# sephiroce/srf

Measured on AMD Instinct MI355X. Metric: acoustic frames/sec through SRF (123-d fbank, 3-iter DR) at 1/2/4/8 MI355X, higher is better.
Workload: dtype fp32; 1 GPU; wsj_c4: SRF L=6 PH=CH=16 DIM=32 LPAD=RPAD=2 DR iter=3, train step (fwd+bwd+allreduce+Adam); utterances_per_gpu=28, frames_per_utterance=800, global_batch=28, parallelism=dp1, launch=hipgraph (fwd+CTC+bwd)

## Files before the change

### srf_amd/csrc/cnnfe.hip

```cpp
#include <algorithm>
#include <type_traits>
#include <cmath>
#include <cstdlib>

#include "srf_common.h"
#include "srf_reduce.h"
#include "srf_rng.h"
#include "../../include/srf.h"

namespace {

constexpr int C = 64;
constexpr float kBnEps = 1e-3f;
constexpr float kBnMomentum = 0.99f;

struct Dims {
  int B, T, Fin;
  int T1, F1, T2, F2;
  int pt1, pf1, pt2, pf2;
};

inline int same_out(int n) { return (n + 1) / 2; }
inline int same_pad_before(int n) {
  const int out = same_out(n);
  const int total = std::max((out - 1) * 2 + 3 - n, 0);
  return total / 2;
}

Dims make_dims(int B, int T, int Fin) {
  Dims d;
  d.B = B; d.T = T; d.Fin = Fin;
  d.T1 = same_out(T); d.F1 = same_out(Fin);
  d.T2 = same_out(d.T1); d.F2 = same_out(d.F1);
  d.pt1 = same_pad_before(T); d.pf1 = same_pad_before(Fin);
  d.pt2 = same_pad_before(d.T1); d.pf2 = same_pad_before(d.F1);
  return d;
}

__device__ __forceinline__ int ceil_div_len(int len, int div) { return (len + div - 1) / div; }

__device__ __forceinline__ void chan_merge(float& n, float& mean, float& m2, float nb, float meanb, float m2b) {
  if (nb == 0.f) return;
  const float nn = n + nb;
  const float delta = meanb - mean;
  mean += delta * (nb / nn);
  m2 += m2b + delta * delta * (n * nb / nn);
  n = nn;
}

constexpr int kPackW2Threads = 2 * C * 64;
constexpr int kPackW2tThreads = 9 * C * (2 * C / 8);
__device__ __forceinline__ void pack_w2_f16_body(int idx, const float* __restrict__ ka, const float* __restrict__ kb,
                                                 _Float16* __restrict__ wp2, float* __restrict__ wsc);
__device__ __forceinline__ void pack_w2t_split_body(int idx, const float* __restrict__ ka,
                                                    const float* __restrict__ kb, __bf16* __restrict__ wq3);
__device__ __forceinline__ void pack_w2t_f16_body(int idx, const float* __restrict__ ka, const float* __restrict__ kb,
                                                  _Float16* __restrict__ wq2h, float* __restrict__ wdsc);
constexpr int kPackW2tF16Threads = C * 64;

constexpr int kRows1 = 4;

struct Tile1 {
  int b, t1_0, fpad;
};

__device__ __forceinline__ Tile1 stage_rows1(const float* __restrict__ feats, const Dims& d, float* win) {
  const int tiles_per_b = (d.T1 + kRows1 - 1) / kRows1;
  Tile1 tl;
  tl.b = blockIdx.x / tiles_per_b;
  tl.t1_0 = (blockIdx.x - tl.b * tiles_per_b) * kRows1;
  tl.fpad = d.Fin + 2;
  const int nrows = 2 * kRows1 + 1;
  const int t_base = 2 * tl.t1_0 - d.pt1;
  for (int k = threadIdx.x; k < nrows * tl.fpad; k += blockDim.x) {
    const int r = k / tl.fpad, col = k - r * tl.fpad;
    const int t = t_base + r, f = col - 1;
    const bool ok = t >= 0 && t < d.T && f >= 0 && f < d.Fin;
    const float v = feats[((size_t)tl.b * d.T + min(max(t, 0), d.T - 1)) * d.Fin + min(max(f, 0), d.Fin - 1)];
    win[k] = ok ? v : 0.f;
  }
  __syncthreads();
  return tl;
}

__device__ __forceinline__ void window9_lds(const float* win, const Tile1& tl, const Dims& d, int w, int f1,
                                            float (&x)[9]) {
#pragma unroll
  for (int dt = 0; dt < 3; ++dt)
#pragma unroll
    for (int df = 0; df < 3; ++df) x[dt * 3 + df] = win[(2 * w + dt) * tl.fpad + 2 * f1 - d.pf1 + df + 1];
}

__global__ __launch_bounds__(256) void conv1_fwd_kernel(
    const float* __restrict__ feats, const int* __restrict__ inp_len, Dims d, const float* __restrict__ ka,
    const float* __restrict__ ba, const float* __restrict__ kb, const float* __restrict__ bb, int training,
    float drop_p, unsigned long long seed, const unsigned long long* __restrict__ seed_src, float* __restrict__ y1, unsigned char* __restrict__ sel1,
    float* __restrict__ part, int nconv, const float* __restrict__ pk_a, const float* __restrict__ pk_b,
    _Float16* __restrict__ wp2, float* __restrict__ wsc, float* __restrict__ ymax) {
  if ((int)blockIdx.x >= nconv) {
    const int idx = (blockIdx.x - nconv) * blockDim.x + threadIdx.x;
    if (idx < kPackW2Threads) pack_w2_f16_body(idx, pk_a, pk_b, wp2, wsc);
    return;
  }
  seed = srf_step_seed(seed, seed_src);
  extern __shared__ __attribute__((aligned(16))) float win[];
  __shared__ float sh[3][kRows1][C];
  const int c = threadIdx.x & (C - 1);
  const int w = __builtin_amdgcn_readfirstlane(threadIdx.x >> 6);
  float wa[9], wb[9];
#pragma unroll
  for (int k = 0; k < 9; ++k) {
    wa[k] = ka[k * C + c];
    wb[k] = kb[k * C + c];
  }
  const float bia = ba[c], bib = bb[c];
  const float keep_scale = 1.f / (1.f - drop_p);
  const bool drop = training && drop_p > 0.f;
  const Tile1 tl = stage_rows1(feats, d, win);
  const int t1 = tl.t1_0 + w;
  float n = 0.f, s1 = 0.f, s2 = 0.f, ym = 0.f;
  const float K = 0.5f * (bia + bib);
  if (t1 < d.T1) {
    const bool live = t1 < ceil_div_len(inp_len[tl.b], 2);
    const int pbase = (tl.b * d.T1 + t1) * d.F1;
#pragma unroll 2
    for (int f1 = 0; f1 < d.F1; ++f1) {
      float x[9];
      window9_lds(win, tl, d, w, f1, x);
      float a = bia, bv = bib;
#pragma unroll
      for (int k = 0; k < 9; ++k) {
        a += x[k] * wa[k];
        bv += x[k] * wb[k];
      }
      const int o = (pbase + f1) * C + c;
      if (drop) {
        bool ka, kb;
        srf_keep2(seed, kStreamConv0a, o, drop_p, ka, kb);
        a *= ka ? keep_scale : 0.f;
        bv *= kb ? keep_scale : 0.f;
      }
      const bool sl = a >= bv;
      const float y = live ? (sl ? a : bv) : 0.f;
      y1[o] = y;
      sel1[o] = sl ? 1 : 0;
      ym = fmaxf(ym, fabsf(y));
      n += 1.f;
      s1 += y - K;
      s2 += (y - K) * (y - K);
    }
  }
  float mean = n > 0.f ? K + s1 / n : 0.f;
  float m2 = n > 0.f ? fmaxf(s2 - s1 * s1 / n, 0.f) : 0.f;
  sh[0][w][c] = n; sh[1][w][c] = mean; sh[2][w][c] = m2;
#pragma unroll
  for (int o = 32; o >= 1; o >>= 1) ym = fmaxf(ym, __shfl_xor(ym, o, 64));
  __shared__ float smax[kRows1];
  if (c == 0) smax[w] = ym;
  __syncthreads();
  if (w == 0) {
    if (c == 0) {
      float m = smax[0];
      for (int r = 1; r < kRows1; ++r) m = fmaxf(m, smax[r]);
      ymax[blockIdx.x] = m;
    }
    for (int r = 1; r < kRows1; ++r) chan_merge(n, mean, m2, sh[0][r][c], sh[1][r][c], sh[2][r][c]);
    part[((size_t)blockIdx.x * 3 + 0) * C + c] = n;
    part[((size_t)blockIdx.x * 3 + 1) * C + c] = mean;
    part[((size_t)blockIdx.x * 3 + 2) * C + c] = m2;
  }
}

__global__ __launch_bounds__(256) void bn_merge_kernel(const float* __restrict__ part, int nparts, int per,
                                                       float* __restrict__ out) {
  __shared__ float sh[3][4][C];
  const int c = threadIdx.x & (C - 1), r = threadIdx.x >> 6;
  const int k0 = blockIdx.x * per, k1 = min(nparts, k0 + per);
  float n = 0.f, mu = 0.f, m2 = 0.f;
  for (int k = k0 + r; k < k1; k += 4)
    chan_merge(n, mu, m2, part[((size_t)k * 3 + 0) * C + c], part[((size_t)k * 3 + 1) * C + c],
               part[((size_t)k * 3 + 2) * C + c]);
  sh[0][r][c] = n; sh[1][r][c] = mu; sh[2][r][c] = m2;
  __syncthreads();
  if (r != 0) return;
  for (int q = 1; q < 4; ++q) chan_merge(n, mu, m2, sh[0][q][c], sh[1][q][c], sh[2][q][c]);
  out[((size_t)blockIdx.x * 3 + 0) * C + c] = n;
  out[((size_t)blockIdx.x * 3 + 1) * C + c] = mu;
  out[((size_t)blockIdx.x * 3 + 2) * C + c] = m2;
}

__global__ __launch_bounds__(1024) void bn_finalize_kernel(const float* __restrict__ part, int nparts,
                                                           const float* __restrict__ gamma,
                                                           const float* __restrict__ beta,
                                                           float* __restrict__ mmean, float* __restrict__ mvar,
                                                           int training, float* __restrict__ stats,
                                                           const float* __restrict__ ymax, int nymax) {
  __shared__ float sh[3][16][C];
  __shared__ float ysh[16], ab[2][C];
  const int c = threadIdx.x & (C - 1), r = threadIdx.x >> 6;
  if (ymax != nullptr) {
    float m = 0.f;
    for (int k = threadIdx.x; k < nymax; k += 1024) m = fmaxf(m, ymax[k]);
#pragma unroll
    for (int o = 32; o >= 1; o >>= 1) m = fmaxf(m, __shfl_xor(m, o, 64));
    if (c == 0) ysh[r] = m;
  }
  float n = 0.f, mu = 0.f, m2 = 0.f;
  if (training)
#pragma unroll 8
    for (int k = r; k < nparts; k += 16)
      chan_merge(n, mu, m2, part[((size_t)k * 3 + 0) * C + c], part[((size_t)k * 3 + 1) * C + c],
                 part[((size_t)k * 3 + 2) * C + c]);
  sh[0][r][c] = n; sh[1][r][c] = mu; sh[2][r][c] = m2;
  __syncthreads();
  if (r == 0) {
    float mean, var;
    if (training) {
      for (int q = 1; q < 16; ++q) chan_merge(n, mu, m2, sh[0][q][c], sh[1][q][c], sh[2][q][c]);
      mean = mu;
      var = m2 / n;
      mmean[c] = mmean[c] * kBnMomentum + mean * (1.f - kBnMomentum);
      mvar[c] = mvar[c] * kBnMomentum + (n > 1.f ? var * n / (n - 1.f) : var) * (1.f - kBnMomentum);
    } else {
      mean = mmean[c];
      var = mvar[c];
    }
    const float rstd = 1.f / sqrtf(var + kBnEps);
    const float scale = gamma[c] * rstd;
    const float shift = beta[c] - mean * scale;
    stats[0 * C + c] = mean;
    stats[1 * C + c] = rstd;
    stats[2 * C + c] = scale;
    stats[3 * C + c] = shift;
    ab[0][c] = fabsf(scale);
    ab[1][c] = fabsf(shift);
  }
  if (ymax == nullptr) return;
  __syncthreads();
  if (threadIdx.x == 0) {
    float y = ysh[0], sa = 0.f, sb = 0.f;
    for (int q = 1; q < 16; ++q) y = fmaxf(y, ysh[q]);
    for (int q = 0; q < C; ++q) {
      sa = fmaxf(sa, ab[0][q]);
      sb = fmaxf(sb, ab[1][q]);
    }
    const int e = srf_split_exp(sa * y + sb);
    stats[4 * C + 0] = srf_exp2i(e);
    stats[4 * C + 1] = srf_exp2i(-e);
  }
}

typedef __bf16 cbf8 __attribute__((ext_vector_type(8)));
typedef float cf16 __attribute__((ext_vector_type(16)));

__device__ __forceinline__ cf16 mfma32bf(const cbf8& a, const cbf8& b, const cf16& c) {
  return __builtin_amdgcn_mfma_f32_32x32x16_bf16(a, b, c, 0, 0, 0);
}
typedef _Float16 ch8 __attribute__((ext_vector_type(8)));
__device__ __forceinline__ cf16 mfma32h(const ch8& a, const ch8& b, const cf16& c) {
  return __builtin_amdgcn_mfma_f32_32x32x16_f16(a, b, c, 0, 0, 0);
}

__device__ __forceinline__ void split8v(const float (&v)[8], cbf8& p1, cbf8& p2, cbf8& p3) {
#pragma unroll
  for (int k = 0; k < 8; ++k) {
    const __bf16 a1 = (__bf16)v[k];
    const float r = v[k] - (float)a1;
    const __bf16 a2 = (__bf16)r;
    p1[k] = a1;
    p2[k] = a2;
    p3[k] = (__bf16)(r - (float)a2);
  }
}

__device__ __forceinline__ void pack_w2_f16_body(int idx, const float* __restrict__ ka, const float* __restrict__ kb,
                                                 _Float16* __restrict__ wp2, float* __restrict__ wsc) {
  const int n = idx >> 6, cin = idx & 63;
  const float* k = n < C ? ka : kb;
  const int co = n % C;
  float v[9], m = 0.f;
#pragma unroll
  for (int tap = 0; tap < 9; ++tap) {
    v[tap] = k[((size_t)tap * C + cin) * C + co];
    m = fmaxf(m, fabsf(v[tap]));
  }
#pragma unroll
  for (int o = 32; o >= 1; o >>= 1) m = fmaxf(m, __shfl_xor(m, o, 64));
  const int e = srf_split_exp(m);
  const float sc = srf_exp2i(e);
  const size_t plane = (size_t)9 * 2 * C * C;
#pragma unroll
  for (int tap = 0; tap < 9; ++tap) {
    _Float16 h1, h2;
    srf_split2h(v[tap] * sc, h1, h2);
    const size_t o = ((size_t)tap * 2 * C + n) * C + cin;
    wp2[o] = h1;
    wp2[plane + o] = h2;
  }
  if (cin == 0) wsc[n] = srf_exp2i(-e);
}

constexpr int kC2BStride = 24;
constexpr int kC2Waves = 4;
constexpr int kC2Px = 32 * kC2Waves;
constexpr int kC2BLoads = 2 * 2 * C * 2 / (64 * kC2Waves);

__global__ __launch_bounds__(64 * kC2Waves) __attribute__((amdgpu_waves_per_eu(2))) void conv2_fwd32_kernel(
    const float* __restrict__ y1, const float* __restrict__ stats1, const int* __restrict__ inp_len, Dims d,
    const _Float16* __restrict__ wp2, const float* __restrict__ wsc, const float* __restrict__ ba,
    const float* __restrict__ bb, int training, float drop_p, unsigned long long seed,
    const unsigned long long* __restrict__ seed_src, float* __restrict__ y2, unsigned char* __restrict__ sel2,
    float* __restrict__ part) {
  seed = srf_step_seed(seed, seed_src);
  __shared__ __attribute__((aligned(16))) _Float16 Bs[2][2][2 * C * kC2BStride];
  __shared__ __attribute__((aligned(16))) float ss[2][C];
  __shared__ float red[3][kC2Waves][2 * 32];
  const int tid = threadIdx.x;
  const int lane = tid & 63, wv = tid >> 6;
  const int r = lane & 31, h = lane >> 5;
  const int P2 = d.B * d.T2 * d.F2;
  const int p0 = blockIdx.x * kC2Px;
  const size_t plane = (size_t)9 * 2 * C * C;
  if (tid < 2 * C) ss[tid >> 6][tid & 63] = stats1[(2 + (tid >> 6)) * C + (tid & 63)] * stats1[4 * C];

  const int pa = p0 + 32 * wv + r;
  const bool alive = pa < P2;
  const int pc = min(pa, P2 - 1);
  const int af2 = pc % d.F2, at2 = (pc / d.F2) % d.T2, ab = pc / (d.F2 * d.T2);
  const int alen1 = ceil_div_len(inp_len[ab], 2);

  auto load_b = [&](int kk, ch8 (&bv)[kC2BLoads]) {
    const int tap = kk >> 2, kb = kk & 3;
#pragma unroll
    for (int q = 0; q < kC2BLoads; ++q) {
      const int idx = q * 64 * kC2Waves + tid;
      const int pl = idx >> 8, rem = idx & 255, n = rem >> 1, half = rem & 1;
      bv[q] = *reinterpret_cast<const ch8*>(wp2 + pl * plane + ((size_t)tap * 2 * C + n) * C + 16 * kb + 8 * half);
    }
  };
  auto store_b = [&](int buf, const ch8 (&bv)[kC2BLoads]) {
#pragma unroll
    for (int q = 0; q < kC2BLoads; ++q) {
      const int idx = q * 64 * kC2Waves + tid;
      const int pl = idx >> 8, rem = idx & 255, n = rem >> 1, half = rem & 1;
      *reinterpret_cast<ch8*>(&Bs[buf][pl][n * kC2BStride + 8 * half]) = bv[q];
    }
  };
  auto load_a = [&](int kk, f4 (&av)[2], bool& ok) {
    const int tap = kk >> 2, kb = kk & 3;
    const int dt = tap / 3, df = tap - dt * 3;
    const int t1 = 2 * at2 - d.pt2 + dt, f1 = 2 * af2 - d.pf2 + df;
    ok = alive && t1 >= 0 && t1 < d.T1 && f1 >= 0 && f1 < d.F1 && t1 < alen1;
    const int t1c = min(max(t1, 0), d.T1 - 1), f1c = min(max(f1, 0), d.F1 - 1);
    const float* src = y1 + (((size_t)ab * d.T1 + t1c) * d.F1 + f1c) * C + 16 * kb + 8 * h;
    av[0] = *reinterpret_cast<const f4*>(src);
    av[1] = *reinterpret_cast<const f4*>(src + 4);
  };

  cf16 acc[4];
#pragma unroll
  for (int nt = 0; nt < 4; ++nt) acc[nt] = cf16{};
  auto compute = [&](int kk, int buf, const f4 (&av)[2], bool aok) {
    ch8 a1, a2;
    {
      const int c0 = 16 * (kk & 3) + 8 * h;
#pragma unroll
      for (int q = 0; q < 8; ++q) {
        const float x = q < 4 ? av[0][q] : av[1][q - 4];
        _Float16 h1, h2;
        srf_split2h(aok ? x * ss[0][c0 + q] + ss[1][c0 + q] : 0.f, h1, h2);
        a1[q] = h1;
        a2[q] = h2;
      }
    }
#pragma unroll
    for (int nt = 0; nt < 4; ++nt) {
      const int nrow = (nt >> 1) * C + 32 * (nt & 1) + r;
      const ch8 b1 = *reinterpret_cast<const ch8*>(&Bs[buf][0][nrow * kC2BStride + 8 * h]);
      const ch8 b2 = *reinterpret_cast<const ch8*>(&Bs[buf][1][nrow * kC2BStride + 8 * h]);
      cf16 c = acc[nt];
      c = mfma32h(a2, b1, c);
      c = mfma32h(a1, b2, c);
      c = mfma32h(a1, b1, c);
      acc[nt] = c;
    }
  };
  ch8 bvA[kC2BLoads], bvB[kC2BLoads];
  f4 avA[2], avB[2], avC[2];
  bool okA, okB, okC;
  load_b(0, bvA);
  load_a(0, avA, okA);
  load_b(1, bvB);
  load_a(1, avB, okB);
  store_b(0, bvA);
  __syncthreads();
  for (int kk = 0; kk < 36; kk += 2) {
    {
      const f4 a0[2] = {avA[0], avA[1]};
      const bool ok0 = okA;
      if (kk + 2 < 36) {
        load_b(kk + 2, bvA);
        load_a(kk + 2, avA, okA);
      }
      compute(kk, 0, a0, ok0);
      store_b(1, bvB);
      __syncthreads();
    }
    {
      const f4 a1v[2] = {avB[0], avB[1]};
      const bool ok1 = okB;
      if (kk + 3 < 36) {
        load_b(kk + 3, bvB);
        load_a(kk + 3, avB, okB);
      }
      compute(kk + 1, 1, a1v, ok1);
      if (kk + 2 < 36) store_b(0, bvA);
      __syncthreads();
    }
  }
  (void)avC;
  (void)okC;

  const float keep_scale = 1.f / (1.f - drop_p);
  const float inv_b = stats1[4 * C + 1];
#pragma unroll
  for (int g = 0; g < 2; ++g) {
    const int c = 32 * g + r;
    const float bia = ba[c], bib = bb[c];
    const float sca = wsc[c] * inv_b, scb = wsc[C + c] * inv_b;
    float n = 0.f, mean = 0.f, m2 = 0.f;
#pragma unroll
    for (int q = 0; q < 4; ++q)
#pragma unroll
      for (int v = 0; v < 4; ++v) {
        const int p = p0 + 32 * wv + 8 * q + 4 * h + v;
        if (p >= P2) continue;
        const int t2 = (p / d.F2) % d.T2, b = p / (d.F2 * d.T2);
        const size_t o = (size_t)p * C + c;
        float a = acc[g][4 * q + v] * sca + bia, bvv = acc[2 + g][4 * q + v] * scb + bib;
        if (training && drop_p > 0.f) {
          bool ka, kb;
          srf_keep2(seed, kStreamConv1a, o, drop_p, ka, kb);
          a *= ka ? keep_scale : 0.f;
          bvv *= kb ? keep_scale : 0.f;
        }
        const bool sel = a >= bvv;
        float y = sel ? a : bvv;
        if (t2 >= ceil_div_len(inp_len[b], 4)) y = 0.f;
        y2[o] = y;
        sel2[o] = sel ? 1 : 0;
        n += 1.f;
        const float delta = y - mean;
        mean += delta / n;
        m2 += delta * (y - mean);
      }
    {
      float nb, mb, qb, x;
      xpair32(n, x, nb);
      nb = h ? x : nb;
      xpair32(mean, x, mb);
      mb = h ? x : mb;
      xpair32(m2, x, qb);
      qb = h ? x : qb;
      if (h == 0) chan_merge(n, mean, m2, nb, mb, qb);
    }
    if (h == 0) {
      red[0][wv][g * 32 + r] = n;
      red[1][wv][g * 32 + r] = mean;
      red[2][wv][g * 32 + r] = m2;
    }
  }
  __syncthreads();
  if (tid < 2 * 32) {
    const int gc = tid;
    float n = red[0][0][gc], mean = red[1][0][gc], m2 = red[2][0][gc];
#pragma unroll
    for (int w = 1; w < kC2Waves; ++w) chan_merge(n, mean, m2, red[0][w][gc], red[1][w][gc], red[2][w][gc]);
    part[((size_t)blockIdx.x * 3 + 0) * C + gc] = n;
    part[((size_t)blockIdx.x * 3 + 1) * C + gc] = mean;
    part[((size_t)blockIdx.x * 3 + 2) * C + gc] = m2;
  }
}

__global__ void bn_apply_kernel(const float* __restrict__ y, const float* __restrict__ stats,
                                const int* __restrict__ inp_len, int B, int Tk, int Fk, int div,
                                float* __restrict__ out) {
  const int n4 = B * Tk * Fk * C / 4;
  for (int q = blockIdx.x * blockDim.x + threadIdx.x; q < n4; q += gridDim.x * blockDim.x) {
    const int c4 = (q * 4) % C;
    const int p = q * 4 / C;
    const int t = (p / Fk) % Tk;
    const int b = p / (Fk * Tk);
    f4 v = {0.f, 0.f, 0.f, 0.f};
    if (t < ceil_div_len(inp_len[b], div)) {
      const f4 x = reinterpret_cast<const f4*>(y)[q];
      v = x * *reinterpret_cast<const f4*>(stats + 2 * C + c4) + *reinterpret_cast<const f4*>(stats + 3 * C + c4);
    }
    reinterpret_cast<f4*>(out)[q] = v;
  }
}


constexpr int kBnPx = 16;
__device__ __forceinline__ f4 wave_sum_px(f4 v) {
#pragma unroll
  for (int o = 16; o <= 32; o <<= 1) {
    v.x += __shfl_xor(v.x, o, 64); v.y += __shfl_xor(v.y, o, 64);
    v.z += __shfl_xor(v.z, o, 64); v.w += __shfl_xor(v.w, o, 64);
  }
  return v;
}

__global__ __launch_bounds__(256) void bn_bwd_reduce_kernel(const float* __restrict__ g, const float* __restrict__ y,
                                                            const float* __restrict__ stats,
                                                            const int* __restrict__ inp_len, int B, int Tk, int Fk,
                                                            int div, float* __restrict__ part) {
  __shared__ f4 sh[2][4][C / 4];
  const int lane = threadIdx.x & 63, q = lane & 15, pg = lane >> 4;
  const int wave = __builtin_amdgcn_readfirstlane(threadIdx.x >> 6);
  const f4 mean = reinterpret_cast<const f4*>(stats)[q], rstd = reinterpret_cast<const f4*>(stats + C)[q];
  const int P = B * Tk * Fk;
  f4 s0 = {0.f, 0.f, 0.f, 0.f}, s1 = s0;
  for (int p0 = (blockIdx.x * 4 + wave) * kBnPx; p0 < P; p0 += gridDim.x * 4 * kBnPx) {
    constexpr int U = kBnPx / 4;
    f4 dy[U], yv[U];
    float m[U];
#pragma unroll
    for (int u = 0; u < U; ++u) {
      const int pu = p0 + 4 * u + pg;
      const int p = min(pu, P - 1);
      const int t = (p / Fk) % Tk;
      const int b = p / (Fk * Tk);
      m[u] = (pu < P && t < ceil_div_len(inp_len[b], div)) ? 1.f : 0.f;
      dy[u] = reinterpret_cast<const f4*>(g)[(size_t)p * (C / 4) + q];
      yv[u] = reinterpret_cast<const f4*>(y)[(size_t)p * (C / 4) + q];
    }
#pragma unroll
    for (int u = 0; u < U; ++u) {
      const f4 d = dy[u] * m[u];
      s0 += d;
      s1 += d * (yv[u] - mean) * rstd;
    }
  }
  s0 = wave_sum_px(s0);
  s1 = wave_sum_px(s1);
  if (pg == 0) { sh[0][wave][q] = s0; sh[1][wave][q] = s1; }
  __syncthreads();
  if (threadIdx.x < 2 * (C / 4)) {
    const int k = threadIdx.x / (C / 4), qq = threadIdx.x % (C / 4);
    const f4 v = sh[k][0][qq] + sh[k][1][qq] + sh[k][2][qq] + sh[k][3][qq];
    reinterpret_cast<f4*>(part + ((size_t)blockIdx.x * 2 + k) * C)[qq] = v;
  }
}

__device__ __forceinline__ float bn_bwd_elem(float gin, float y, float mask, float mean, float rstd, float gamma,
                                             float sdy_n, float sdyxh_n) {
  const float dy = mask * gin;
  const float xh = (y - mean) * rstd;
  return mask * gamma * rstd * (dy - sdy_n - xh * sdyxh_n);
}

__global__ __launch_bounds__(256) void conv2_bwd_prep_kernel(
    const float* __restrict__ g_out, const float* __restrict__ y2, const unsigned char* __restrict__ sel2,
    const float* __restrict__ stats2, const float* __restrict__ gamma2, const float* __restrict__ bnsum2,
    const int* __restrict__ inp_len, Dims d, float drop_p, unsigned long long seed, const unsigned long long* __restrict__ seed_src, float* __restrict__ g_ab,
    float* __restrict__ part, int nprep, const float* __restrict__ pk_a, const float* __restrict__ pk_b,
    __bf16* __restrict__ wq3, _Float16* __restrict__ wq2h, float* __restrict__ wdsc, float* __restrict__ gmax) {
  if ((int)blockIdx.x >= nprep) {
    const int idx = (blockIdx.x - nprep) * blockDim.x + threadIdx.x;
    if (wq2h != nullptr) {
      if (idx < kPackW2tF16Threads) pack_w2t_f16_body(idx, pk_a, pk_b, wq2h, wdsc);
    } else if (idx < kPackW2tThreads) {
      pack_w2t_split_body(idx, pk_a, pk_b, wq3);
    }
    return;
  }
  seed = srf_step_seed(seed, seed_src);
  __shared__ f4 sh[2][4][C / 4];
  __shared__ float smax[4];
  const int lane = threadIdx.x & 63, q = lane & 15, pg = lane >> 4;
  const int wave = __builtin_amdgcn_readfirstlane(threadIdx.x >> 6);
  const int P = d.B * d.T2 * d.F2;
  const f4 mean = reinterpret_cast<const f4*>(stats2)[q], rstd = reinterpret_cast<const f4*>(stats2 + C)[q];
  const f4 gam = {gamma2[4 * q], gamma2[4 * q + 1], gamma2[4 * q + 2], gamma2[4 * q + 3]};
  const f4 sdy_n = reinterpret_cast<const f4*>(bnsum2)[q] / (float)P;
  const f4 sdyxh_n = reinterpret_cast<const f4*>(bnsum2 + C)[q] / (float)P;
  const float keep_scale = 1.f / (1.f - drop_p);
  f4 ga_s = {0.f, 0.f, 0.f, 0.f}, gb_s = ga_s;
  float gm = 0.f;
  for (int p0 = (blockIdx.x * 4 + wave) * kBnPx; p0 < P; p0 += nprep * 4 * kBnPx) {
    constexpr int U = kBnPx / 4;
    f4 gv[U], yv[U];
    unsigned sv[U];
    float m[U];
#pragma unroll
    for (int u = 0; u < U; ++u) {
      const int pu = p0 + 4 * u + pg;
      const int p = min(pu, P - 1);
      const int t = (p / d.F2) % d.T2;
      const int b = p / (d.F2 * d.T2);
      m[u] = (pu < P && t < ceil_div_len(inp_len[b], 4)) ? 1.f : 0.f;
      gv[u] = reinterpret_cast<const f4*>(g_out)[(size_t)p * (C / 4) + q];
      yv[u] = reinterpret_cast<const f4*>(y2)[(size_t)p * (C / 4) + q];
// ... 565 lines not shown
    }
  }
#pragma unroll
  for (int j = 0; j < 20; ++j) sh[w][j][c] = acc[j];
  __syncthreads();
  for (int j = w; j < 20; j += kRows1) {
    float v = 0.f;
#pragma unroll
    for (int r = 0; r < kRows1; ++r) v += sh[r][j][c];
    part[((size_t)blockIdx.x * 20 + j) * C + c] = v;
  }
}

inline int conv1_blocks(const Dims& d) { return d.B * ((d.T1 + kRows1 - 1) / kRows1); }
inline size_t conv1_lds(const Dims& d) { return (size_t)(2 * kRows1 + 1) * (d.Fin + 2) * sizeof(float); }

struct FwdSaved {
  float *y1, *y2, *stats1, *stats2;
  unsigned char *sel1, *sel2;
  size_t bytes;
};

FwdSaved saved_layout(const Dims& d, void* base) {
  const size_t P1 = (size_t)d.B * d.T1 * d.F1, P2 = (size_t)d.B * d.T2 * d.F2;
  size_t off = 0;
  auto take = [&](size_t bytes) {
    size_t o = off;
    off += srf::align_up(bytes, 256);
    return o;
  };
  const size_t oy1 = take(P1 * C * 4), oy2 = take(P2 * C * 4), os1 = take(5 * C * 4), os2 = take(5 * C * 4),
               osel1 = take(P1 * C), osel2 = take(P2 * C);
  char* b = static_cast<char*>(base);
  FwdSaved s;
  s.y1 = (float*)(b + oy1);
  s.y2 = (float*)(b + oy2);
  s.stats1 = (float*)(b + os1);
  s.stats2 = (float*)(b + os2);
  s.sel1 = (unsigned char*)(b + osel1);
  s.sel2 = (unsigned char*)(b + osel2);
  s.bytes = off;
  return s;
}

constexpr int kBnMerge = 32;

int bn_finalize(const float* part, int nparts, float* merged, const float* gamma, const float* beta, float* mmean,
                float* mvar, int training, float* stats, hipStream_t st, const float* ymax = nullptr,
                int nymax = 0) {
  const int per = (nparts + kBnMerge - 1) / kBnMerge;
  hipLaunchKernelGGL(bn_merge_kernel, dim3(kBnMerge), dim3(256), 0, st, part, nparts, per, merged);
  SRF_LAUNCH_CHECK("bn_merge");
  hipLaunchKernelGGL(bn_finalize_kernel, dim3(1), dim3(1024), 0, st, merged, kBnMerge, gamma, beta, mmean, mvar,
                     training, stats, ymax, nymax);
  SRF_LAUNCH_CHECK("bn_finalize");
  return SRF_OK;
}

struct FwdWs {
  float *part1, *part2, *wp, *merged;
  _Float16* wp2;
  float* wsc;
  float* ymax;
  size_t bytes;
};

FwdWs fwd_ws_layout(const Dims& d, void* base) {
  const size_t P2 = (size_t)d.B * d.T2 * d.F2;
  const size_t nb2 = (P2 + 63) / 64;
  size_t off = 0;
  auto take = [&](size_t bytes) {
    size_t o = off;
    off += srf::align_up(bytes, 256);
    return o;
  };
  const size_t op1 = take((size_t)conv1_blocks(d) * 3 * C * 4), op2 = take(nb2 * 3 * C * 4),
               owp = take((size_t)9 * 2 * C * C * 4), omg = take((size_t)kBnMerge * 3 * C * 4),
               owp2 = take((size_t)2 * 9 * 2 * C * C * 2), owsc = take((size_t)2 * C * 4),
               oym = take((size_t)conv1_blocks(d) * 4);
  char* b = static_cast<char*>(base);
  FwdWs w;
  w.wp2 = (_Float16*)(b + owp2);
  w.wsc = (float*)(b + owsc);
  w.ymax = (float*)(b + oym);
  w.merged = (float*)(b + omg);
  w.part1 = (float*)(b + op1);
  w.part2 = (float*)(b + op2);
  w.wp = (float*)(b + owp);
  w.bytes = off;
  return w;
}

int check_dims(int B, int T, int Fin, int nfilt) {
  SRF_REQUIRE(B > 0 && T > 0 && Fin > 0, "bad CNN-FE shape B=%d T=%d F=%d", B, T, Fin);
  SRF_REQUIRE(nfilt == C, "model-conv-filter-num must be %d (got %d)", C, nfilt);
  return SRF_OK;
}

}

extern "C" {

int srf_cnnfe_out_dims(int T, int feat_dim, int* T2, int* F2) {
  SRF_REQUIRE(T > 0 && feat_dim > 0 && T2 && F2, "bad arguments");
  Dims d = make_dims(1, T, feat_dim);
  *T2 = d.T2;
  *F2 = d.F2;
  return SRF_OK;
}

size_t srf_cnnfe_saved_bytes(int B, int T, int feat_dim, int nfilt) {
  (void)nfilt;
  return saved_layout(make_dims(B, T, feat_dim), nullptr).bytes;
}

size_t srf_cnnfe_fwd_workspace(int B, int T, int feat_dim, int nfilt) {
  (void)nfilt;
  return fwd_ws_layout(make_dims(B, T, feat_dim), nullptr).bytes;
}

int srf_cnnfe_fwd(const float* feats, const int* inp_len, int B, int T, int feat_dim, int nfilt,
                  const float* k0a, const float* b0a, const float* k0b, const float* b0b, const float* gamma0,
                  const float* beta0, const float* k1a, const float* b1a, const float* k1b, const float* b1b,
                  const float* gamma1, const float* beta1, float* mmean0, float* mvar0, float* mmean1, float* mvar1,
                  int training, float drop_p, unsigned long long seed, float* out, void* saved, size_t saved_bytes,
                  void* workspace, size_t workspace_bytes, void* stream) {
  int rc = check_dims(B, T, feat_dim, nfilt);
  if (rc) return rc;
  SRF_REQUIRE(feats && inp_len && k0a && b0a && k0b && b0b && gamma0 && beta0 && k1a && b1a && k1b && b1b &&
                  gamma1 && beta1 && mmean0 && mvar0 && mmean1 && mvar1 && out && saved && workspace,
              "null pointer argument");
  SRF_REQUIRE(drop_p >= 0.f && drop_p < 1.f, "dropout rate %f out of [0,1)", drop_p);
  const Dims d = make_dims(B, T, feat_dim);
  FwdSaved sv = saved_layout(d, saved);
  FwdWs w = fwd_ws_layout(d, workspace);
  if (saved_bytes < sv.bytes || workspace_bytes < w.bytes) {
    srf::set_error("CNN-FE buffers too small (saved %zu < %zu or workspace %zu < %zu)", saved_bytes, sv.bytes,
                   workspace_bytes, w.bytes);
    return SRF_EWORKSPACE;
  }
  hipStream_t st = static_cast<hipStream_t>(stream);
  const size_t P2 = (size_t)d.B * d.T2 * d.F2;
  const int nb2 = (int)((P2 + 63) / 64);
  int nparts2 = nb2;
  const int npack = (kPackW2Threads + 64 * kRows1 - 1) / (64 * kRows1);
  hipLaunchKernelGGL(conv1_fwd_kernel, dim3(conv1_blocks(d) + npack), dim3(64 * kRows1), conv1_lds(d), st, feats,
                     inp_len, d, k0a, b0a, k0b, b0b, training, drop_p, seed, srf::seed_source(), sv.y1, sv.sel1,
                     w.part1, conv1_blocks(d), k1a, k1b, w.wp2, w.wsc, w.ymax);
  SRF_LAUNCH_CHECK("conv1_fwd");
  if ((rc = bn_finalize(w.part1, conv1_blocks(d), w.merged, gamma0, beta0, mmean0, mvar0, training, sv.stats1, st,
                        w.ymax, conv1_blocks(d))))
    return rc;
  SRF_LAUNCH_CHECK("bn_finalize(1)");
  {
    const int nb32 = (int)((P2 + kC2Px - 1) / kC2Px);
    hipLaunchKernelGGL(conv2_fwd32_kernel, dim3(nb32), dim3(64 * kC2Waves), 0, st, sv.y1, sv.stats1, inp_len, d,
                       w.wp2, w.wsc, b1a, b1b, training, drop_p, seed, srf::seed_source(), sv.y2, sv.sel2,
                       w.part2);
    SRF_LAUNCH_CHECK("conv2_fwd32");
    nparts2 = nb32;
  }
  if ((rc = bn_finalize(w.part2, nparts2, w.merged, gamma1, beta1, mmean1, mvar1, training, sv.stats2, st)))
    return rc;
  SRF_LAUNCH_CHECK("bn_finalize(2)");
  hipLaunchKernelGGL(bn_apply_kernel, dim3(1024), dim3(256), 0, st, sv.y2, sv.stats2, inp_len, d.B, d.T2, d.F2, 4,
                     out);
  SRF_LAUNCH_CHECK("bn_apply");
  return SRF_OK;
}

}

namespace {
struct BwdWs2 {
  float *bnpart, *bnsum2, *bnsum1, *g_ab, *biaspart, *g_x1, *wq, *wpart, *c1part, *c1sum, *scratch;
  __bf16* gsT3;
  float* gmax;
  float* wdsc;
  int P2p;
  size_t bytes;
};

constexpr int kBnBlocks = 1024;
constexpr int kWgrad32SplitsMax = 128;
constexpr int kWgrad32Splits = 56;

BwdWs2 bwd_ws_layout(const Dims& d, void* base) {
  const size_t P1 = (size_t)d.B * d.T1 * d.F1, P2 = (size_t)d.B * d.T2 * d.F2;
  size_t off = 0;
  auto take = [&](size_t bytes) {
    size_t o = off;
    off += srf::align_up(bytes, 256);
    return o;
  };
  const size_t obp = take((size_t)kBnBlocks * 2 * C * 4), os2 = take(2 * C * 4), os1 = take(2 * C * 4),
               oab = take(P2 * 2 * C * 4), obias = take((size_t)kBnBlocks * 2 * C * 4), ogx = take(P1 * C * 4),
               owq = take((size_t)9 * 2 * C * C * 4), owp = take((size_t)kWgrad32SplitsMax * 9 * C * 2 * C * 4),
               oc1 = take((size_t)conv1_blocks(d) * 20 * C * 4), oc1s = take(20 * C * 4),
               oscr = take(srf::colsum_scratch_floats(std::max(conv1_blocks(d), kBnBlocks), 20 * C) * 4);
  const int P2p = (int)((P2 + kTpPx - 1) / kTpPx * kTpPx);
  const size_t ogs3 = take((size_t)3 * 2 * C * P2p * 2);
  const size_t ogm = take((size_t)kBnBlocks * 4), ods = take((size_t)C * 4);
  char* b = static_cast<char*>(base);
  BwdWs2 w;
  w.bnpart = (float*)(b + obp);
  w.bnsum2 = (float*)(b + os2);
  w.bnsum1 = (float*)(b + os1);
  w.g_ab = (float*)(b + oab);
  w.biaspart = (float*)(b + obias);
  w.g_x1 = (float*)(b + ogx);
  w.wq = (float*)(b + owq);
  w.wpart = (float*)(b + owp);
  w.c1part = (float*)(b + oc1);
  w.c1sum = (float*)(b + oc1s);
  w.scratch = (float*)(b + oscr);
  w.gsT3 = (__bf16*)(b + ogs3);
  w.gmax = (float*)(b + ogm);
  w.wdsc = (float*)(b + ods);
  w.P2p = P2p;
  w.bytes = off;
  return w;
}

}

extern "C" {

size_t srf_cnnfe_bwd_workspace(int B, int T, int feat_dim, int nfilt) {
  (void)nfilt;
  return bwd_ws_layout(make_dims(B, T, feat_dim), nullptr).bytes;
}

int srf_cnnfe_bwd(const float* feats, const int* inp_len, int B, int T, int feat_dim, int nfilt, const float* gamma0,
                  const float* k1a, const float* k1b, const float* gamma1, float drop_p, unsigned long long seed,
                  const void* saved, const float* g_out, float* g_k0a, float* g_b0a, float* g_k0b, float* g_b0b,
                  float* g_gamma0, float* g_beta0, float* g_k1a, float* g_b1a, float* g_k1b, float* g_b1b,
                  float* g_gamma1, float* g_beta1, void* workspace, size_t workspace_bytes, void* stream) {
  return srf_cnnfe_bwd_parts(SRF_CNNFE_BWD_ALL, feats, inp_len, B, T, feat_dim, nfilt, gamma0, k1a, k1b, gamma1, drop_p,
                             seed, saved, g_out, g_k0a, g_b0a, g_k0b, g_b0b, g_gamma0, g_beta0, g_k1a, g_b1a, g_k1b,
                             g_b1b, g_gamma1, g_beta1, workspace, workspace_bytes, stream);
}

int srf_cnnfe_bwd_parts(int parts, const float* feats, const int* inp_len, int B, int T, int feat_dim, int nfilt,
                        const float* gamma0, const float* k1a, const float* k1b, const float* gamma1, float drop_p,
                        unsigned long long seed, const void* saved, const float* g_out, float* g_k0a, float* g_b0a,
                        float* g_k0b, float* g_b0b, float* g_gamma0, float* g_beta0, float* g_k1a, float* g_b1a,
                        float* g_k1b, float* g_b1b, float* g_gamma1, float* g_beta1, void* workspace,
                        size_t workspace_bytes, void* stream) {
  SRF_REQUIRE(parts > 0 && (parts & ~SRF_CNNFE_BWD_ALL) == 0, "CNN-FE backward: bad parts mask %d", parts);
  int rc = check_dims(B, T, feat_dim, nfilt);
  if (rc) return rc;
  SRF_REQUIRE(feats && inp_len && gamma0 && k1a && k1b && gamma1 && saved && g_out && g_k0a && g_b0a && g_k0b &&
                  g_b0b && g_gamma0 && g_beta0 && g_k1a && g_b1a && g_k1b && g_b1b && g_gamma1 && g_beta1 &&
                  workspace,
              "null pointer argument");
  SRF_REQUIRE(((uintptr_t)g_out & 15) == 0 && ((uintptr_t)saved & 255) == 0 && ((uintptr_t)workspace & 255) == 0,
              "CNN-FE backward: g_out must be 16-byte and saved / workspace 256-byte aligned");
  const Dims d = make_dims(B, T, feat_dim);
  FwdSaved sv = saved_layout(d, const_cast<void*>(saved));
  BwdWs2 w = bwd_ws_layout(d, workspace);
  if (workspace_bytes < w.bytes) {
    srf::set_error("CNN-FE backward workspace too small: %zu < %zu", workspace_bytes, w.bytes);
    return SRF_EWORKSPACE;
  }
  hipStream_t st = static_cast<hipStream_t>(stream);
  const int P2 = d.B * d.T2 * d.F2;
  __bf16* wq3 = reinterpret_cast<__bf16*>(w.wq);
  _Float16* wq2h = reinterpret_cast<_Float16*>(w.wq);
  if (parts & SRF_CNNFE_BWD_PREP) {
  hipLaunchKernelGGL(bn_bwd_reduce_kernel, dim3(kBnBlocks), dim3(256), 0, st, g_out, sv.y2, sv.stats2, inp_len, d.B,
                     d.T2, d.F2, 4, w.bnpart);
  SRF_LAUNCH_CHECK("bn_bwd_reduce(2)");
  if ((rc = srf::colsum(w.bnpart, kBnBlocks, 2 * C, w.bnsum2, w.scratch, st, srf::ColSplit{{g_beta1, g_gamma1, nullptr, nullptr}, {C, C, 0, 0}})))
    return rc;
  const int npack = (kPackW2tF16Threads + 255) / 256;
  hipLaunchKernelGGL(conv2_bwd_prep_kernel, dim3(kBnBlocks + npack), dim3(256), 0, st, g_out, sv.y2, sv.sel2,
                     sv.stats2, gamma1, w.bnsum2, inp_len, d, drop_p, seed, srf::seed_source(), w.g_ab, w.biaspart,
                     kBnBlocks, k1a, k1b, wq3, wq2h, w.wdsc, w.gmax);
  SRF_LAUNCH_CHECK("conv2_bwd_prep");
  if ((rc = srf::colsum(w.biaspart, kBnBlocks, 2 * C, nullptr, w.scratch, st, srf::ColSplit{{g_b1a, g_b1b, nullptr, nullptr}, {C, C, 0, 0}})))
    return rc;
  }
  if (parts & SRF_CNNFE_BWD_DATA) {
    DgCls cls{};
    for (int c = 0; c < 4; ++c) {
      const int qt = c >> 1, qf = c & 1;
      const int Pc = d.B * ((d.T1 - qt + 1) / 2) * ((d.F1 - qf + 1) / 2);
      cls.boff[c + 1] = cls.boff[c] + (Pc + kD2Px - 1) / kD2Px;
    }
    hipLaunchKernelGGL(conv2_dgrad32_kernel<true>, dim3(cls.boff[4]), dim3(64 * kD2Waves), 0, st, w.g_ab,
                       (const void*)wq2h, d, cls, w.g_x1, (const float*)w.gmax, kBnBlocks, (const float*)w.wdsc);
    SRF_LAUNCH_CHECK("conv2_dgrad32");
  }
  const WgDiv dv{make_fastdiv(d.F2), make_fastdiv(d.T2)};
  const int nsplit = kWgrad32Splits;
  if (parts & SRF_CNNFE_BWD_WGRAD) {
    static_assert(kW2Chunk == kWgChunk, "wgrad splits are whole chunks");
    const int split_len = ((P2 + nsplit - 1) / nsplit + kWgChunk - 1) / kWgChunk * kWgChunk;
    hipLaunchKernelGGL(gab_split_t_kernel<true>, dim3(w.P2p / kTpPx), dim3(256), 0, st, w.g_ab, P2, w.P2p,
                       (void*)w.gsT3, (const float*)w.gmax, kBnBlocks);
    SRF_LAUNCH_CHECK("gab_split_t");
    hipLaunchKernelGGL(conv2_wgrad32_kernel<true>, dim3(9 * nsplit), dim3(256), 0, st, sv.y1, sv.stats1, inp_len,
                       (const void*)w.gsT3, w.P2p, d, dv, nsplit, split_len, w.wpart, (const float*)w.gmax,
                       kBnBlocks);
    SRF_LAUNCH_CHECK("conv2_wgrad32");
    hipLaunchKernelGGL(conv2_wgrad_reduce_kernel, dim3((9 * C * 2 * C + 255) / 256), dim3(256), 0, st, w.wpart,
                       nsplit, g_k1a, g_k1b);
// ... 19 lines not shown
```

Before: 3.028 million frames/s.

## Add patch-based conv2 forward kernel staging input band in LDS

Adds a new conv2 forward kernel that stages a band of BN-normalized, fp16-split input rows into swizzled LDS once per (batch, time-band) block and runs the 3x3 conv as MFMA over that patch. Weights are repacked into an MFMA-friendly tiled layout so each lane loads its fragment directly with deep register prefetch. BN statistics are moved out into a separate partials kernel that rereads y2. This trades redundant global input loads for an extra kernel launch and an extra pass over the output.

Result: no change. 3.045 million frames/s, median of 6 (+0.5%).

```diff
diff --git a/srf_amd/csrc/cnnfe.hip b/srf_amd/csrc/cnnfe.hip
--- a/srf_amd/csrc/cnnfe.hip
+++ b/srf_amd/csrc/cnnfe.hip
@@ -38,6 +38,10 @@
 }
 
 __device__ __forceinline__ int ceil_div_len(int len, int div) { return (len + div - 1) / div; }
+
+#ifndef SRF_CONV2_PATCH
+#define SRF_CONV2_PATCH 1
+#endif
 
 __device__ __forceinline__ void chan_merge(float& n, float& mean, float& m2, float nb, float meanb, float m2b) {
   if (nb == 0.f) return;
@@ -273,6 +277,14 @@
   }
 }
 
+__device__ __forceinline__ size_t wp2_off(int tap, int n, int cin) {
+#if SRF_CONV2_PATCH
+  return (((((size_t)tap * 4 + (cin >> 4)) * 4 + (n >> 5)) * 2 + ((cin >> 3) & 1)) * 32 + (n & 31)) * 8 + (cin & 7);
+#else
+  return ((size_t)tap * 2 * C + n) * C + cin;
+#endif
+}
+
 __device__ __forceinline__ void pack_w2_f16_body(int idx, const float* __restrict__ ka, const float* __restrict__ kb,
                                                  _Float16* __restrict__ wp2, float* __restrict__ wsc) {
   const int n = idx >> 6, cin = idx & 63;
@@ -293,7 +305,7 @@
   for (int tap = 0; tap < 9; ++tap) {
     _Float16 h1, h2;
     srf_split2h(v[tap] * sc, h1, h2);
-    const size_t o = ((size_t)tap * 2 * C + n) * C + cin;
+    const size_t o = wp2_off(tap, n, cin);
     wp2[o] = h1;
     wp2[plane + o] = h2;
   }
@@ -335,7 +347,7 @@
     for (int q = 0; q < kC2BLoads; ++q) {
       const int idx = q * 64 * kC2Waves + tid;
       const int pl = idx >> 8, rem = idx & 255, n = rem >> 1, half = rem & 1;
-      bv[q] = *reinterpret_cast<const ch8*>(wp2 + pl * plane + ((size_t)tap * 2 * C + n) * C + 16 * kb + 8 * half);
+      bv[q] = *reinterpret_cast<const ch8*>(wp2 + pl * plane + wp2_off(tap, n, 16 * kb + 8 * half));
     }
   };
   auto store_b = [&](int buf, const ch8 (&bv)[kC2BLoads]) {
@@ -449,6 +461,232 @@
         if (t2 >= ceil_div_len(inp_len[b], 4)) y = 0.f;
         y2[o] = y;
         sel2[o] = sel ? 1 : 0;
+        n += 1.f;
+        const float delta = y - mean;
+        mean += delta / n;
+        m2 += delta * (y - mean);
+      }
+    {
+      float nb, mb, qb, x;
+      xpair32(n, x, nb);
+      nb = h ? x : nb;
+      xpair32(mean, x, mb);
+      mb = h ? x : mb;
+      xpair32(m2, x, qb);
+      qb = h ? x : qb;
+      if (h == 0) chan_merge(n, mean, m2, nb, mb, qb);
+    }
+    if (h == 0) {
+      red[0][wv][g * 32 + r] = n;
+      red[1][wv][g * 32 + r] = mean;
+      red[2][wv][g * 32 + r] = m2;
+    }
+  }
+  __syncthreads();
+  if (tid < 2 * 32) {
+    const int gc = tid;
+    float n = red[0][0][gc], mean = red[1][0][gc], m2 = red[2][0][gc];
+#pragma unroll
+    for (int w = 1; w < kC2Waves; ++w) chan_merge(n, mean, m2, red[0][w][gc], red[1][w][gc], red[2][w][gc]);
+    part[((size_t)blockIdx.x * 3 + 0) * C + gc] = n;
+    part[((size_t)blockIdx.x * 3 + 1) * C + gc] = mean;
+    part[((size_t)blockIdx.x * 3 + 2) * C + gc] = m2;
+  }
+}
+
+constexpr int kP2Band = 2;
+constexpr int kP2Rows = 2 * kP2Band + 1;
+constexpr int kP2MaxF2 = 32;
+constexpr int kP2Threads = 256;
+constexpr int kP2XchgBytes = 4 * 16 * 64 * 4;
+inline size_t conv2_patch_lds(const Dims& d) {
+  return std::max((size_t)kP2Rows * (2 * d.F2 + 1) * 256, (size_t)kP2XchgBytes);
+}
+inline int conv2_patch_blocks(const Dims& d) { return d.B * ((d.T2 + kP2Band - 1) / kP2Band); }
+inline bool conv2_patch_ok(const Dims& d) { return SRF_CONV2_PATCH && d.F2 <= kP2MaxF2; }
+
+__global__ __launch_bounds__(kP2Threads) void conv2_fwd_patch_kernel(
+    const float* __restrict__ y1, const float* __restrict__ stats1, const int* __restrict__ inp_len, Dims d,
+    const _Float16* __restrict__ wp2, const float* __restrict__ wsc, const float* __restrict__ ba,
+    const float* __restrict__ bb, int training, float drop_p, unsigned long long seed,
+    const unsigned long long* __restrict__ seed_src, float* __restrict__ y2, unsigned char* __restrict__ sel2) {
+  seed = srf_step_seed(seed, seed_src);
+  extern __shared__ __attribute__((aligned(16))) unsigned char img[];
+  const int tid = threadIdx.x;
+  const int lane = tid & 63, w = __builtin_amdgcn_readfirstlane(tid >> 6);
+  const int ab = w >> 1, g = w & 1;
+  const int r = lane & 31, h = lane >> 5;
+  const int nbands = (d.T2 + kP2Band - 1) / kP2Band;
+  const int b = blockIdx.x / nbands, t2_0 = (blockIdx.x - b * nbands) * kP2Band;
+  const int W = 2 * d.F2 + 1;
+  const int t1_0 = 2 * t2_0 - d.pt2;
+  const int len1 = min(ceil_div_len(inp_len[b], 2), d.T1);
+
+  {
+    const int c8 = tid & 7, jt = tid >> 3;
+    float sc[8], sh[8];
+#pragma unroll
+    for (int q = 0; q < 8; ++q) {
+      sc[q] = stats1[2 * C + 8 * c8 + q] * stats1[4 * C];
+      sh[q] = stats1[3 * C + 8 * c8 + q] * stats1[4 * C];
+    }
+    constexpr int U = 2;
+    for (int j0 = jt; j0 < W; j0 += 32 * U) {
+      f4 v[kP2Rows][U][2];
+#pragma unroll
+      for (int i = 0; i < kP2Rows; ++i) {
+        const int t1 = t1_0 + i;
+        if (t1 >= 0 && t1 < len1) {
+          const float* row = y1 + ((size_t)b * d.T1 + t1) * d.F1 * C + 8 * c8;
+#pragma unroll
+          for (int u = 0; u < U; ++u) {
+            const int f1c = min(max(j0 + 32 * u - d.pf2, 0), d.F1 - 1);
+            v[i][u][0] = *reinterpret_cast<const f4*>(row + (size_t)f1c * C);
+            v[i][u][1] = *reinterpret_cast<const f4*>(row + (size_t)f1c * C + 4);
+          }
+        } else {
+#pragma unroll
+          for (int u = 0; u < U; ++u) v[i][u][0] = v[i][u][1] = f4{0.f, 0.f, 0.f, 0.f};
+        }
+      }
+#pragma unroll
+      for (int i = 0; i < kP2Rows; ++i) {
+        const int t1 = t1_0 + i;
+        const bool rowok = t1 >= 0 && t1 < len1;
+#pragma unroll
+        for (int u = 0; u < U; ++u) {
+          const int j = j0 + 32 * u, f1 = j - d.pf2;
+          if (j >= W) continue;
+          const bool ok = rowok && f1 >= 0 && f1 < d.F1;
+          ch8 a1, a2;
+#pragma unroll
+          for (int q = 0; q < 8; ++q) {
+            const float x = q < 4 ? v[i][u][0][q] : v[i][u][1][q - 4];
+            _Float16 h1, h2;
+            srf_split2h(ok ? x * sc[q] + sh[q] : 0.f, h1, h2);
+            a1[q] = h1;
+            a2[q] = h2;
+          }
+          unsigned char* px = img + (size_t)(i * W + j) * 256;
+          const int x = (j >> 1) & 15;
+          *reinterpret_cast<ch8*>(px + ((c8 ^ x) << 4)) = a1;
+          *reinterpret_cast<ch8*>(px + (((8 + c8) ^ x) << 4)) = a2;
+        }
+      }
+    }
+  }
+  __syncthreads();
+
+  const int f2a = min(r, d.F2 - 1);
+  const unsigned char* abase = img + (size_t)(2 * f2a) * 256;
+  const int ysw[2] = {h ^ (f2a & 15), h ^ ((f2a + 1) & 15)};
+  const _Float16* wb = wp2 + (size_t)w * 512 + lane * 8;
+  constexpr size_t plane = (size_t)9 * 2 * C * C;
+  auto load_b = [&](int kk, ch8 (&bv)[2]) {
+#pragma unroll
+    for (int pl = 0; pl < 2; ++pl) bv[pl] = *reinterpret_cast<const ch8*>(wb + pl * plane + (size_t)kk * 4 * 512);
+  };
+  cf16 acc[kP2Band];
+#pragma unroll
+  for (int m = 0; m < kP2Band; ++m) acc[m] = cf16{};
+  auto load_a = [&](int kk, ch8 (&av)[kP2Band][2]) {
+    const int tap = kk >> 2, kb = kk & 3;
+    const int dt = tap / 3, df = tap - dt * 3;
+#pragma unroll
+    for (int m = 0; m < kP2Band; ++m)
+#pragma unroll
+      for (int pl = 0; pl < 2; ++pl)
+        av[m][pl] = *reinterpret_cast<const ch8*>(abase + (size_t)((2 * m + dt) * W + df) * 256 +
+                                                  (((8 * pl + 2 * kb) ^ ysw[df == 2]) << 4));
+  };
+  constexpr int kAhead = 8, kRing = kAhead + 1, kAheadA = 2, kRingA = kAheadA + 1;
+  ch8 bq[kRing][2], aq[kRingA][kP2Band][2];
+#pragma unroll
+  for (int kk = 0; kk < kAhead; ++kk) load_b(kk, bq[kk]);
+#pragma unroll
+  for (int kk = 0; kk < kAheadA; ++kk) load_a(kk, aq[kk]);
+#pragma unroll
+  for (int kk = 0; kk < 36; ++kk) {
+    if (kk + kAhead < 36) load_b(kk + kAhead, bq[(kk + kAhead) % kRing]);
+    if (kk + kAheadA < 36) load_a(kk + kAheadA, aq[(kk + kAheadA) % kRingA]);
+    __builtin_amdgcn_sched_barrier(0);
+#pragma unroll
+    for (int term = 0; term < 3; ++term)
+#pragma unroll
+      for (int m = 0; m < kP2Band; ++m)
+        acc[m] = mfma32h(aq[kk % kRingA][m][term == 0 ? 1 : 0], bq[kk % kRing][term == 1 ? 1 : 0], acc[m]);
+    __builtin_amdgcn_sched_barrier(0);
+  }
+
+  __syncthreads();
+  float* xch = reinterpret_cast<float*>(img);
+#pragma unroll
+  for (int k = 0; k < 16; ++k) xch[(w * 16 + k) * 64 + lane] = ab ? acc[0][k] : acc[1][k];
+  __syncthreads();
+  cf16 ca, cb;
+#pragma unroll
+  for (int k = 0; k < 16; ++k) {
+    const float o = xch[((w ^ 2) * 16 + k) * 64 + lane];
+    ca[k] = ab ? o : acc[0][k];
+    cb[k] = ab ? acc[1][k] : o;
+  }
+
+  const float keep_scale = 1.f / (1.f - drop_p);
+  const float inv_b = stats1[4 * C + 1];
+  const int c = 32 * g + r;
+  const float bia = ba[c], bib = bb[c];
+  const float sca = wsc[c] * inv_b, scb = wsc[C + c] * inv_b;
+  const int len2 = ceil_div_len(inp_len[b], 4);
+  const int t2 = t2_0 + ab;
+  if (t2 < d.T2) {
+#pragma unroll
+    for (int q = 0; q < 4; ++q)
+#pragma unroll
+      for (int v = 0; v < 4; ++v) {
+        const int f2 = 8 * q + 4 * h + v;
+        if (f2 >= d.F2) continue;
+        const size_t o = (((size_t)b * d.T2 + t2) * d.F2 + f2) * C + c;
+        float av = ca[4 * q + v] * sca + bia, bvv = cb[4 * q + v] * scb + bib;
+        if (training && drop_p > 0.f) {
+          bool ka, kb;
+          srf_keep2(seed, kStreamConv1a, o, drop_p, ka, kb);
+          av *= ka ? keep_scale : 0.f;
+          bvv *= kb ? keep_scale : 0.f;
+        }
+        const bool sel = av >= bvv;
+        float y = sel ? av : bvv;
+        if (t2 >= len2) y = 0.f;
+        y2[o] = y;
+        sel2[o] = sel ? 1 : 0;
+      }
+  }
+}
+
+__global__ __launch_bounds__(64 * kC2Waves) void bn2_partials_kernel(const float* __restrict__ y2, int P2,
+                                                                     float* __restrict__ part) {
+  __shared__ float red[3][kC2Waves][2 * 32];
+  const int tid = threadIdx.x;
+  const int lane = tid & 63, wv = tid >> 6;
+  const int r = lane & 31, h = lane >> 5;
+  const int p0 = blockIdx.x * kC2Px;
+  float yv[2][16];
+#pragma unroll
+  for (int g = 0; g < 2; ++g)
+#pragma unroll
+    for (int k = 0; k < 16; ++k) {
+      const int p = min(p0 + 32 * wv + 8 * (k >> 2) + 4 * h + (k & 3), P2 - 1);
+      yv[g][k] = y2[(size_t)p * C + 32 * g + r];
+    }
+#pragma unroll
+  for (int g = 0; g < 2; ++g) {
+    float n = 0.f, mean = 0.f, m2 = 0.f;
+#pragma unroll
+    for (int q = 0; q < 4; ++q)
+#pragma unroll
+      for (int v = 0; v < 4; ++v) {
+        const int p = p0 + 32 * wv + 8 * q + 4 * h + v;
+        if (p >= P2) continue;
+        const float y = yv[g][4 * q + v];
         n += 1.f;
         const float delta = y - mean;
         mean += delta / n;
@@ -1320,7 +1558,20 @@
                         w.ymax, conv1_blocks(d))))
     return rc;
   SRF_LAUNCH_CHECK("bn_finalize(1)");
-  {
+  if (conv2_patch_ok(d)) {
+    const size_t lds = conv2_patch_lds(d);
+    if (lds > 64 * 1024)
+      SRF_HIP_TRY(hipFuncSetAttribute((const void*)conv2_fwd_patch_kernel, hipFuncAttributeMaxDynamicSharedMemorySize,
+                                      (int)lds));
+    hipLaunchKernelGGL(conv2_fwd_patch_kernel, dim3(conv2_patch_blocks(d)), dim3(kP2Threads), lds, st, sv.y1,
+                       sv.stats1, inp_len, d, w.wp2, w.wsc, b1a, b1b, training, drop_p, seed, srf::seed_source(),
+                       sv.y2, sv.sel2);
+    SRF_LAUNCH_CHECK("conv2_fwd_patch");
+    nparts2 = (int)((P2 + kC2Px - 1) / kC2Px);
+    hipLaunchKernelGGL(bn2_partials_kernel, dim3(nparts2), dim3(64 * kC2Waves), 0, st, (const float*)sv.y2, (int)P2,
+                       w.part2);
+    SRF_LAUNCH_CHECK("bn2_partials");
+  } else {
     const int nb32 = (int)((P2 + kC2Px - 1) / kC2Px);
     hipLaunchKernelGGL(conv2_fwd32_kernel, dim3(nb32), dim3(64 * kC2Waves), 0, st, sv.y1, sv.stats1, inp_len, d,
                        w.wp2, w.wsc, b1a, b1b, training, drop_p, seed, srf::seed_source(), sv.y2, sv.sel2,
```
